# LiMeng95/MultiPoseNet.pytorch

Hardware: AMD Instinct MI355X
Metric: images/sec (train fwd+bwd) ResNet101 480x480 bs=32/GPU (higher is better)
Workload: dtype bf16; 1 GPU; R101 full posenet (keypoint+detection) train step: fwd + MSE/focal losses + bwd + Adam, 480x480, 32 images/GPU, bf16 MFMA / fp32 accumulate / fp32 master weights; global_batch=32, parallelism=dp1, loss_log=asynchronous (set_lazy_log), launch=recorded launch list re-issued per step (replay.py), 88 replays, optimizer_update=Adam in one launch after backward

## Files before the change

include/mpn.h:

```cpp
#ifndef MPN_H_
#define MPN_H_
#include <stdint.h>

#ifdef __cplusplus
extern "C" {
#endif

#define MPN_F32 0
#define MPN_BF16 1
#define MPN_F16 2

#define MPN_E_BADARG (-2)
#define MPN_E_UNSUPPORTED (-3)

typedef struct MpnConvParams {
    const void* x;
    const void* w;
    void* y;
    const float* bias;
    const float* scale;
    const void* res;
    const uint8_t* res_mask;
    float* stats;
    int64_t x_sB, x_sH, x_sW;
// ... 73 lines not shown
} MpnWgradParams;
int mpn_debug_wgrad_prof(void* buf);
int mpn_debug_igemm_prof(void* buf);

int mpn_conv_wgrad_chunks(const MpnWgradParams* p);
int mpn_conv_wgrad_seg_plan(MpnWgradParams* p);
int mpn_conv_wgrad(const MpnWgradParams* p, void* stream);
int mpn_conv_wgrad_partials(const MpnWgradParams* p, void* stream);
int mpn_conv_wgrad_reduce(const MpnWgradParams* p, void* stream);
int mpn_conv_wgrad_kernel_id(const MpnWgradParams* p);

int mpn_reduce_partials(const float* ws, int chunks, int64_t n, float* dst, int accumulate, void* stream);

int mpn_cast_f32_to_bf16(const float* src, void* dst, int64_t n, void* stream);
int mpn_cast_f32(const float* src, void* dst, int64_t n, int dtype, void* stream);
int mpn_weight_transpose(const float* w, void* wt, int Cout, int RS, int Cin, int Cout_pad,
                         int dtype, void* stream);
int mpn_weight_transpose_batched(const float* arena, void* dst, const int64_t* table, int nlayers, int64_t nblocks,
                                 int dtype, void* stream);
int mpn_weight_pad_k(const float* w, void* dst, int Cout, int K, int Kpad, int dtype, void* stream);
int mpn_stem_pack_weight(const float* w, void* packed, int Cout, int dtype, void* stream);
int mpn_stem_unpack_wgrad(const float* dpacked, float* dw, int Cout, void* stream);
int mpn_stem_pack_image(const float* img, int64_t sB, int64_t sC, int64_t sH, int64_t sW, void* dst,
                        int B, int H, int W, int dtype, void* stream);

int mpn_bn_finalize_train(const float* stats, int tiles, int C, int64_t count, const float* gamma,
                          const float* beta, float* running_mean, float* running_var, float momentum,
                          float eps, float* mean, float* invstd, float* scale, float* shift, void* stream);
int mpn_bn_finalize_eval(int C, const float* gamma, const float* beta, const float* running_mean,
                         const float* running_var, float eps, float* mean, float* invstd,
                         float* scale, float* shift, void* stream);
int mpn_bn_act_forward(const void* y, const void* res, void* z, const float* scale, const float* shift,
                       int64_t P, int C, int Cs, int relu, int dtype, uint8_t* mask, void* stream);
int mpn_bn_bwd_reduce(const void* dz, const void* z, const void* y, const float* mean, const float* invstd,
                      const float* mask_scale, const float* mask_shift, float* partial, int chunks, int64_t P, int C, int Cs, int relu, int dtype, void* stream);
int mpn_bn_bwd_finalize(const float* partial, int chunks, int C, int64_t count, const float* gamma, const float* mean,
                        const float* invstd, int train, float* dgamma, float* dbeta, float* coef, void* stream);
int mpn_bn_bwd_apply(const void* dz, const void* z, const void* y, const float* k1, const float* k2, const float* k3,
                     const float* mask_scale, const float* mask_shift, void* dy, void* dres, int dres_accumulate, int64_t P, int C, int Cs, int relu, int dtype,
                     const uint8_t* mask, void* stream);
int mpn_bn_bwd_chunks(int64_t P, int Cs, int dtype);

int mpn_maxpool3x3s2_forward(const void* x, void* y, uint8_t* idx, int B, int H, int W, int Cs,
                             int Ho, int Wo, int dtype, void* stream);
int mpn_maxpool3x3s2_backward(const void* dy, const uint8_t* idx, void* dx, int B, int H, int W, int Cs,
                              int Ho, int Wo, int dtype, void* stream);
int mpn_upsample_nearest_backward(const void* dfine, void* dcoarse, int B, int Hf, int Wf, int Hc, int Wc,
                                  int Cs, int accumulate, int dtype, void* stream);
int mpn_upsample_nearest_slice(const void* src, void* dst, int B, int Hs, int Ws, int Cs_src,
                               int Ho, int Wo, int Cs_dst, int c_off, int dtype, void* stream);
int mpn_upsample_nearest_slice_backward(const void* ddst, void* dsrc, int B, int Hs, int Ws, int Cs_src,
                                        int Ho, int Wo, int Cs_dst, int c_off, int dtype, void* stream);
int mpn_export_f32(const void* src, int src_dtype, float* dst, int B, int Hs, int Ws, int Cs, int C,
                   int Ho, int Wo, int64_t dst_sB, int64_t dst_sP, void* stream);
int mpn_import_grad(const float* ddst, int64_t ddst_sB, int64_t ddst_sP, void* dsrc, int dst_dtype,
                    int B, int Hs, int Ws, int Cs, int C, int Ho, int Wo, void* stream);
int mpn_nchw_to_nhwc_f32(const float* src, int64_t sB, int64_t sC, int64_t sH, int64_t sW, float* dst,
                         int B, int C, int H, int W, void* stream);
int mpn_det_pack(const void* src, int src_dtype, float* dst, int B, int64_t HW, int Cs, int C, int64_t dst_sB, void* stream);
int mpn_det_unpack(const float* ddst, void* dsrc, int dst_dtype, int B, int64_t HW, int Cs, int C, int64_t dst_sB, void* stream);
int mpn_relu_forward(const void* x, void* y, int64_t n, int dtype, void* stream);
int mpn_relu_backward(const void* dz, const void* z, void* dx, int64_t n, int accumulate, int dtype, void* stream);
int mpn_add_inplace(void* dst, const void* src, int64_t n, int dtype, void* stream);
int mpn_channel_sum(const void* dy, int dy_dtype, int64_t P, int C, int Cs, float* partial, int chunks, void* stream);
int mpn_channel_sum_chunks(int64_t P, int Cs, int dtype);
int mpn_colsum_rows(const void* dy, int dy_dtype, int64_t P, int C, int Cs, float* db, void* stream);
// ... 112 lines not shown
```

multiposenet/pytorch_amd/_lib.py:

```python
import ctypes
import os
import subprocess

import torch

_HERE = os.path.dirname(os.path.abspath(__file__))
LIB_PATH = os.path.join(_HERE, "libmpn_hip.so")
CSRC = os.path.join(_HERE, "csrc")

F32, BF16, F16 = 0, 1, 2


class MpnError(RuntimeError):
    pass


class ConvParams(ctypes.Structure):
    _fields_ = [
        ("x", ctypes.c_void_p), ("w", ctypes.c_void_p), ("y", ctypes.c_void_p),
        ("bias", ctypes.c_void_p), ("scale", ctypes.c_void_p), ("res", ctypes.c_void_p), ("res_mask", ctypes.c_void_p),
        ("stats", ctypes.c_void_p),
        ("x_sB", ctypes.c_int64), ("x_sH", ctypes.c_int64), ("x_sW", ctypes.c_int64),
        ("y_sB", ctypes.c_int64), ("y_sP", ctypes.c_int64),
        ("res_sB", ctypes.c_int64), ("res_sP", ctypes.c_int64),
# ... 38 lines not shown
SIGNATURES = {
    "mpn_gt_heatmaps": (_i, [_vp, _vp, _i, _i, _vp, _i, _i, ctypes.c_double, ctypes.c_double, _vp]),
    "mpn_heatmap_peaks_workspace_bytes": (_i64, [_i, _i, _i, _i, _i]),
    "mpn_heatmap_peaks": (_i, [_vp, _i64, _i64, _i64, _i64, _i, _i, _i, _i, _f, ctypes.c_double, _i, _vp, _vp, _i, _vp, _vp]),
    "mpn_resize": (_i, [_vp, _i64, _i64, _i64, _i, _i, _i, _vp, _i, _i, _i, ctypes.c_double, ctypes.c_double, _vp]),
    "mpn_prn_build_maps": (_i, [_vp, _vp, _vp, _vp, _i, _i, _i, ctypes.c_double, _vp, _vp, _vp, _vp, _vp]),
    "mpn_prn_scores": (_i, [_vp, _vp, _i, _i, _i, _i, _vp, _vp, _vp]),
    "mpn_prn_scores_compact": (_i, [_vp, _vp, _i, _i, _i, _i, _i, _vp, _vp, _vp, _vp, _vp, _vp]),
    "mpn_prn_match_host": (_i, [_i, _vp, _vp, _vp, _vp, _vp, _vp, _vp, _i, _vp, _i, _i, _vp, _vp]),
    "mpn_conv_stats_tiles": (_i, [_PC]),
    "mpn_conv_tile_rows": (_i, [_PC]),
    "mpn_conv_shared_tile": (_i, [_PC]),
    "mpn_conv_forward": (_i, [_PC, _vp]),
    "mpn_debug_wgrad_prof": (_i, [_vp]),
    "mpn_debug_igemm_prof": (_i, [_vp]),
    "mpn_conv_wgrad_chunks": (_i, [_PW]),
    "mpn_conv_wgrad_seg_plan": (_i, [_PW]),
    "mpn_conv_wgrad": (_i, [_PW, _vp]),
    "mpn_conv_wgrad_partials": (_i, [_PW, _vp]),
    "mpn_conv_wgrad_reduce": (_i, [_PW, _vp]),
    "mpn_conv_wgrad_kernel_id": (_i, [_PW]),
    "mpn_reduce_partials": (_i, [_vp, _i, _i64, _vp, _i, _vp]),
    "mpn_cast_f32_to_bf16": (_i, [_vp, _vp, _i64, _vp]),
    "mpn_cast_f32": (_i, [_vp, _vp, _i64, _i, _vp]),
    "mpn_weight_transpose": (_i, [_vp, _vp, _i, _i, _i, _i, _i, _vp]),
    "mpn_weight_transpose_batched": (_i, [_vp, _vp, _vp, _i, _i64, _i, _vp]),
    "mpn_weight_pad_k": (_i, [_vp, _vp, _i, _i, _i, _i, _vp]),
    "mpn_stem_pack_weight": (_i, [_vp, _vp, _i, _i, _vp]),
    "mpn_stem_unpack_wgrad": (_i, [_vp, _vp, _i, _vp]),
    "mpn_stem_pack_image": (_i, [_vp, _i64, _i64, _i64, _i64, _vp, _i, _i, _i, _i, _vp]),
    "mpn_bn_finalize_train": (_i, [_vp, _i, _i, _i64, _vp, _vp, _vp, _vp, _f, _f, _vp, _vp, _vp, _vp, _vp]),
    "mpn_bn_finalize_eval": (_i, [_i, _vp, _vp, _vp, _vp, _f, _vp, _vp, _vp, _vp, _vp]),
    "mpn_bn_act_forward": (_i, [_vp, _vp, _vp, _vp, _vp, _i64, _i, _i, _i, _i, _vp, _vp]),
    "mpn_bn_bwd_reduce": (_i, [_vp, _vp, _vp, _vp, _vp, _vp, _vp, _vp, _i, _i64, _i, _i, _i, _i, _vp]),
    "mpn_bn_bwd_finalize": (_i, [_vp, _i, _i, _i64, _vp, _vp, _vp, _i, _vp, _vp, _vp, _vp]),
    "mpn_bn_bwd_apply": (_i, [_vp, _vp, _vp, _vp, _vp, _vp, _vp, _vp, _vp, _vp, _i, _i64, _i, _i, _i, _i, _vp, _vp]),
    "mpn_bn_bwd_chunks": (_i, [_i64, _i, _i]),
    "mpn_maxpool3x3s2_forward": (_i, [_vp, _vp, _vp, _i, _i, _i, _i, _i, _i, _i, _vp]),
    "mpn_maxpool3x3s2_backward": (_i, [_vp, _vp, _vp, _i, _i, _i, _i, _i, _i, _i, _vp]),
    "mpn_upsample_nearest_backward": (_i, [_vp, _vp, _i, _i, _i, _i, _i, _i, _i, _i, _vp]),
    "mpn_upsample_nearest_slice": (_i, [_vp, _vp, _i, _i, _i, _i, _i, _i, _i, _i, _i, _vp]),
    "mpn_upsample_nearest_slice_backward": (_i, [_vp, _vp, _i, _i, _i, _i, _i, _i, _i, _i, _i, _vp]),
    "mpn_export_f32": (_i, [_vp, _i, _vp, _i, _i, _i, _i, _i, _i, _i, _i64, _i64, _vp]),
    "mpn_import_grad": (_i, [_vp, _i64, _i64, _vp, _i, _i, _i, _i, _i, _i, _i, _i, _vp]),
    "mpn_nchw_to_nhwc_f32": (_i, [_vp, _i64, _i64, _i64, _i64, _vp, _i, _i, _i, _i, _vp]),
    "mpn_det_pack": (_i, [_vp, _i, _vp, _i, _i64, _i, _i, _i64, _vp]),
    "mpn_det_unpack": (_i, [_vp, _vp, _i, _i, _i64, _i, _i, _i64, _vp]),
    "mpn_relu_forward": (_i, [_vp, _vp, _i64, _i, _vp]),
    "mpn_relu_backward": (_i, [_vp, _vp, _vp, _i64, _i, _i, _vp]),
    "mpn_add_inplace": (_i, [_vp, _vp, _i64, _i, _vp]),
    "mpn_channel_sum": (_i, [_vp, _i, _i64, _i, _i, _vp, _i, _vp]),
    "mpn_colsum_rows": (_i, [_vp, _i, _i64, _i, _i, _vp, _vp]),
    "mpn_channel_sum_chunks": (_i, [_i64, _i, _i]),
    "mpn_mse_chunks": (_i, [_i64]),
    "mpn_mse_heatmap_forward": (_i, [_vp, _vp, _vp, _vp, _i64, _vp, _i, _vp, _vp]),
    "mpn_mse_heatmap_backward": (_i, [_vp, _vp, _vp, _vp, _vp, _vp, _vp, _i64, _vp, _vp]),
    "mpn_mse_train_blocks": (_i, [_i, _i, _i]),
    "mpn_mse_heatmap_train": (_i, [_vp, _vp, _vp, _i, _vp, _vp, _i64, _i64, _i64, _i, _i, _i, _vp, _vp, _i, _vp, _vp]),
    "mpn_focal_blocks": (_i, [_i]),
    "mpn_focal_forward": (_i, [_vp, _vp, _vp, _vp, _i, _i, _i, _vp, _vp, _vp, _vp]),
    "mpn_focal_backward": (_i, [_vp, _vp, _vp, _vp, _i, _i, _i, _vp, _vp, _vp, _vp, _vp]),
    "mpn_focal_mc_blocks": (_i, [_i]),
    "mpn_focal_forward_mc": (_i, [_vp, _vp, _vp, _vp, _i, _i, _i, _i, _vp, _vp, _vp, _vp, _vp]),
    "mpn_focal_backward_mc": (_i, [_vp, _vp, _vp, _vp, _i, _i, _i, _i, _vp, _vp, _vp, _vp, _vp]),
    "mpn_class_max": (_i, [_vp, _i, _i, _i, _vp, _vp, _vp]),
    "mpn_sigmoid_forward": (_i, [_vp, _vp, _i64, _vp]),
# ... 117 lines not shown
```

multiposenet/pytorch_amd/csrc/bn.hip:

```cpp
#include "common.h"
#include <stdlib.h>

namespace {

template <typename T> struct Geo {
    static constexpr int V = Vec16<T>::N;
    int G, GB, lanes, g, pl, c0;
    __device__ __forceinline__ Geo(int Cs) {
        G = Cs / V;
        GB = G < 256 ? G : 256;
        lanes = 256 / GB;
        g = blockIdx.y * GB + (threadIdx.x % GB);
        pl = threadIdx.x / GB;
        c0 = g * V;
    }
};

template <int V>
__device__ __forceinline__ void load_coef(const float* __restrict__ p, int c0, int C, float (&out)[V], float fill) {
#pragma unroll
    for (int k = 0; k < V; k += 4) {
        if (p != nullptr && c0 + k + 3 < C) {
            const float4 t = *reinterpret_cast<const float4*>(p + c0 + k);
            out[k] = t.x; out[k + 1] = t.y; out[k + 2] = t.z; out[k + 3] = t.w;
        } else {
#pragma unroll
            for (int j = 0; j < 4; ++j) out[k + j] = (p != nullptr && c0 + k + j < C) ? p[c0 + k + j] : fill;
        }
    }
}

__device__ __forceinline__ void reduce_slices(const float* __restrict__ part, int n, int C, int c, int sl, double& s1, double& s2) {
    const float* col = part + (long)c * 2;
    const long stride = (long)C * 2;
    int t = sl;
    for (; t + 7 * 64 < n; t += 8 * 64) {
        float2 v[8];
#pragma unroll
        for (int u = 0; u < 8; ++u) v[u] = *reinterpret_cast<const float2*>(col + (long)(t + u * 64) * stride);
#pragma unroll
        for (int u = 0; u < 8; ++u) { s1 += (double)v[u].x; s2 += (double)v[u].y; }
    }
    float2 w[8];
    int m = 0;
#pragma unroll
    for (int u = 0; u < 8; ++u) {
        const int tt = t + u * 64;
        w[u] = tt < n ? *reinterpret_cast<const float2*>(col + (long)tt * stride) : make_float2(0.f, 0.f);
        m += tt < n ? 1 : 0;
    }
#pragma unroll
    for (int u = 0; u < 8; ++u) if (u < m) { s1 += (double)w[u].x; s2 += (double)w[u].y; }
}

__device__ __forceinline__ void finalize_train_block(int blk, const float* __restrict__ stats, int tiles, int C, double count,
                                                     const float* __restrict__ gamma, const float* __restrict__ beta,
                                                     float* __restrict__ rm, float* __restrict__ rv, float momentum, float eps,
                                                     float* __restrict__ mean, float* __restrict__ invstd,
                                                     float* __restrict__ scale, float* __restrict__ shift, double (*sh)[4][4]) {
    const int cl = threadIdx.x & 3, sl = threadIdx.x >> 2;
    const int c = blk * 4 + cl;
    double s1 = 0.0, s2 = 0.0;
    const bool fin = sl == 0 && c < C;
    const float g = (fin && gamma) ? gamma[c] : 1.f, b = (fin && beta) ? beta[c] : 0.f;
    const float rm0 = (fin && rm) ? rm[c] : 0.f, rv0 = (fin && rv) ? rv[c] : 0.f;
    if (c < C) reduce_slices(stats, tiles, C, c, sl, s1, s2);
#pragma unroll
    for (int m = 4; m < 64; m <<= 1) { s1 += __shfl_xor(s1, m); s2 += __shfl_xor(s2, m); }
    const int lane = threadIdx.x & 63, wave = threadIdx.x >> 6;
    if (lane < 4) { sh[0][wave][cl] = s1; sh[1][wave][cl] = s2; }
    __syncthreads();
    if (sl == 0 && c < C) {
        s1 = (sh[0][0][cl] + sh[0][1][cl]) + (sh[0][2][cl] + sh[0][3][cl]);
        s2 = (sh[1][0][cl] + sh[1][1][cl]) + (sh[1][2][cl] + sh[1][3][cl]);
        const double mu = s1 / count;
        double var = s2 / count - mu * mu;
        if (var < 0.0) var = 0.0;
        const float is = (float)(1.0 / sqrt(var + (double)eps));
        const float sc = g * is;
        mean[c] = (float)mu; invstd[c] = is;
        scale[c] = sc; shift[c] = b - (float)mu * sc;
        if (rm) rm[c] = (1.f - momentum) * rm0 + momentum * (float)mu;
        if (rv) {
            const double unb = count > 1.0 ? var * count / (count - 1.0) : var;
            rv[c] = (1.f - momentum) * rv0 + momentum * (float)unb;
        }
    }
}

__global__ void bn_finalize_train_kernel(const float* __restrict__ stats, int tiles, int C, double count,
                                         const float* __restrict__ gamma, const float* __restrict__ beta,
                                         float* __restrict__ rm, float* __restrict__ rv, float momentum, float eps,
                                         float* __restrict__ mean, float* __restrict__ invstd,
                                         float* __restrict__ scale, float* __restrict__ shift) {
    __shared__ double sh[2][4][4];
    finalize_train_block(blockIdx.x, stats, tiles, C, count, gamma, beta, rm, rv, momentum, eps, mean, invstd, scale, shift, sh);
}

__global__ void bn_finalize_eval_kernel(int C, const float* __restrict__ gamma, const float* __restrict__ beta,
                                        const float* __restrict__ rm, const float* __restrict__ rv, float eps,
                                        float* __restrict__ mean, float* __restrict__ invstd,
                                        float* __restrict__ scale, float* __restrict__ shift) {
    const int c = blockIdx.x * blockDim.x + threadIdx.x;
    if (c >= C) return;
    const float is = 1.0f / sqrtf(rv[c] + eps);
    const float sc = gamma[c] * is;
    mean[c] = rm[c]; invstd[c] = is; scale[c] = sc; shift[c] = beta[c] - rm[c] * sc;
}

template <typename T>
__global__ void __launch_bounds__(256) bn_act_kernel(const T* __restrict__ y, const T* __restrict__ res, T* __restrict__ z,
                                                     const float* __restrict__ scale, const float* __restrict__ shift,
                                                     long P, int C, int Cs, int relu, int iters, unsigned char* __restrict__ mask) {
    constexpr int V = Vec16<T>::N;
    const Geo<T> q(Cs);
    float sc[V], sf[V];
    load_coef<V>(scale, q.c0, C, sc, 0.f);
    load_coef<V>(shift, q.c0, C, sf, 0.f);
    const long p0 = (long)blockIdx.x * q.lanes * iters + q.pl;
    for (int it = 0; it < iters; ++it) {
        const long p = p0 + (long)it * q.lanes;
        if (p >= P) break;
        const long off = p * Cs + q.c0;
        Vec16<T> a; a.load(y + off);
        Vec16<T> r;
        if (res) r.load(res + off);
#pragma unroll
        for (int k = 0; k < V; ++k) {
            float x = a.v[k] * sc[k] + sf[k];
            if (res) x += r.v[k];
            if (relu) x = fmaxf(x, 0.f);
            a.v[k] = (q.c0 + k < C) ? x : 0.f;
        }
        a.store(z + off);
        if (mask) {
            unsigned bits = 0;
#pragma unroll
            for (int k = 0; k < V; ++k) bits |= (Elem<T>::round(a.v[k]) > 0.f ? 1u : 0u) << k;
            mask[p * q.G + q.g] = (unsigned char)bits;
        }
    }
}

template <typename T>
__global__ void __launch_bounds__(256) bn_bwd_reduce_kernel(const T* __restrict__ dz, const T* __restrict__ z, const T* __restrict__ y,
                                                            const float* __restrict__ mean, const float* __restrict__ invstd,
                                                            const float* __restrict__ mscale, const float* __restrict__ mshift,
                                                            float* __restrict__ partial, long P, int C, int Cs, int relu, int chunk_pix) {
    constexpr int V = Vec16<T>::N;
    __shared__ float sh[256][2 * V + 1];
    const Geo<T> q(Cs);
    const long p_begin = (long)blockIdx.x * chunk_pix;
    long p_end = p_begin + chunk_pix; if (p_end > P) p_end = P;
    float s1[V], s2[V], mu[V], is[V], sc[V], sf[V];
    load_coef<V>(mean, q.c0, C, mu, 0.f);
    load_coef<V>(invstd, q.c0, C, is, 0.f);
    const bool remask = relu && z == nullptr;
    if (remask) { load_coef<V>(mscale, q.c0, C, sc, 0.f); load_coef<V>(mshift, q.c0, C, sf, 0.f); }
#pragma unroll
    for (int k = 0; k < V; ++k) { s1[k] = 0.f; s2[k] = 0.f; }
    for (long p = p_begin + q.pl; p < p_end; p += q.lanes) {
        const long off = p * Cs + q.c0;
        Vec16<T> d, o, x;
        d.load(dz + off); x.load(y + off);
        if (relu && !remask) o.load(z + off);
#pragma unroll
        for (int k = 0; k < V; ++k) {
            float gk = d.v[k];
            if (remask) o.v[k] = x.v[k] * sc[k] + sf[k];
            if (relu && !(o.v[k] > 0.f)) gk = 0.f;
            s1[k] += gk;
            s2[k] += gk * ((x.v[k] - mu[k]) * is[k]);
        }
// ... 113 lines not shown

}

extern "C" int mpn_bn_finalize_train(const float* stats, int tiles, int C, int64_t count, const float* gamma,
                                     const float* beta, float* running_mean, float* running_var, float momentum,
                                     float eps, float* mean, float* invstd, float* scale, float* shift, void* stream) {
    MPN_CHECK_ARG(stats && tiles > 0 && C > 0 && count > 0 && mean && invstd && scale && shift);
    hipLaunchKernelGGL(bn_finalize_train_kernel, dim3((C + 3) / 4), dim3(256), 0, (hipStream_t)stream, stats, tiles, C,
                       (double)count, gamma, beta, running_mean, running_var, momentum, eps, mean, invstd, scale, shift);
    return mpn_launch_status();
}

extern "C" int mpn_bn_finalize_eval(int C, const float* gamma, const float* beta, const float* running_mean,
                                    const float* running_var, float eps, float* mean, float* invstd,
                                    float* scale, float* shift, void* stream) {
    MPN_CHECK_ARG(C > 0 && gamma && beta && running_mean && running_var && mean && invstd && scale && shift);
    hipLaunchKernelGGL(bn_finalize_eval_kernel, dim3((C + 255) / 256), dim3(256), 0, (hipStream_t)stream, C, gamma, beta,
                       running_mean, running_var, eps, mean, invstd, scale, shift);
    return mpn_launch_status();
}

extern "C" int mpn_bn_act_forward(const void* y, const void* res, void* z, const float* scale, const float* shift,
                                  int64_t P, int C, int Cs, int relu, int dtype, uint8_t* mask, void* stream) {
    MPN_CHECK_ARG(y && z && scale && shift && P > 0 && C > 0 && Cs >= C && (!mask || relu));
    const int V = dtype == MPN_F32 ? 4 : 8;
    MPN_CHECK_ARG(geo_ok(Cs, V) && C % 4 == 0);
    const int lanes = geo_lanes(Cs, V), iters = pick_iters(P, lanes);
    dim3 grid((unsigned)((P + (long)lanes * iters - 1) / ((long)lanes * iters)), (unsigned)geo_yblocks(Cs, V));
    MPN_DISPATCH_T(dtype, hipLaunchKernelGGL((bn_act_kernel<T>), grid, dim3(256), 0, (hipStream_t)stream, (const T*)y, (const T*)res,
                           (T*)z, scale, shift, (long)P, C, Cs, relu, iters, (unsigned char*)mask));
    return mpn_launch_status();
}

extern "C" int mpn_bn_bwd_chunks(int64_t P, int Cs, int dtype) {
    const int V = dtype == MPN_F32 ? 4 : 8;
    if (!geo_ok(Cs, V) || P <= 0) return MPN_E_BADARG;
    const int chunk = reduce_chunk(P, geo_lanes(Cs, V));
    return (int)((P + chunk - 1) / chunk);
}

extern "C" int mpn_bn_bwd_reduce(const void* dz, const void* z, const void* y, const float* mean, const float* invstd,
                                 const float* mask_scale, const float* mask_shift, float* partial, int chunks, int64_t P, int C, int Cs, int relu, int dtype, void* stream) {
    MPN_CHECK_ARG(dz && y && mean && invstd && partial && P > 0 && C > 0 && Cs >= C);
    MPN_CHECK_ARG(!relu || z || (mask_scale && mask_shift && y));
    const int V = dtype == MPN_F32 ? 4 : 8;
    MPN_CHECK_ARG(geo_ok(Cs, V) && C % 4 == 0);
    const int chunk = reduce_chunk(P, geo_lanes(Cs, V));
    MPN_CHECK_ARG(chunks == (int)((P + chunk - 1) / chunk));
    dim3 grid((unsigned)chunks, (unsigned)geo_yblocks(Cs, V));
    MPN_DISPATCH_T(dtype, hipLaunchKernelGGL((bn_bwd_reduce_kernel<T>), grid, dim3(256), 0, (hipStream_t)stream, (const T*)dz, (const T*)z,
                           (const T*)y, mean, invstd, mask_scale, mask_shift, partial, (long)P, C, Cs, relu, chunk));
    return mpn_launch_status();
}

extern "C" int mpn_bn_bwd_finalize(const float* partial, int chunks, int C, int64_t count, const float* gamma, const float* mean,
                                   const float* invstd, int train, float* dgamma, float* dbeta, float* coef, void* stream) {
    MPN_CHECK_ARG(partial && chunks > 0 && C > 0 && count > 0);
    MPN_CHECK_ARG(!coef || (mean && invstd));
    hipLaunchKernelGGL(bn_bwd_finalize_kernel, dim3((C + 3) / 4), dim3(256), 0, (hipStream_t)stream, partial, chunks, C,
                       (double)count, gamma, mean, invstd, train, dgamma, dbeta, coef);
    return mpn_launch_status();
}

extern "C" int mpn_bn_bwd_apply(const void* dz, const void* z, const void* y, const float* k1, const float* k2, const float* k3,
                                const float* mask_scale, const float* mask_shift, void* dy, void* dres, int dres_accumulate, int64_t P, int C, int Cs, int relu, int dtype,
                                const uint8_t* mask, void* stream) {
// ... 14 lines not shown
```

multiposenet/pytorch_amd/engine.py:

```python
import ctypes
import os

import torch

from . import ops
from ._lib import MpnError, call, gpu_op
from .ops import Act, round_up


class Ctx(object):

    def __init__(self, train):
        self.train = train
        self.tape = []
        self.grads = {}
        self.keep = []
        self.out_grads = {}
        self.wt = {}
        self.wt_buf = None
        self.uses = {}
        self.bn_train_ran = False
        self.side_keep = []
        self.side_pending = []
        self.wt_ready = None
# ... 19 lines not shown
        self.grads[id(act)] = g
        self.keep.append(act)

    def pop_grad(self, act):
        return self.grads.pop(id(act), None)


def num_classes(cm):
    cout = cm.output.weight.shape[0]
    if cout % 9 != 0 or cout == 0 or getattr(cm, "num_anchors", 9) != 9:
        raise MpnError("classificationModel: the output convolution has %d channels; the detector needs 9 anchors x K classes" % cout)
    return cout // 9


def _geom(layer):
    w = layer.weight
    if w.dim() == 2:
        return w.shape[0], w.shape[1], 1, 1, 1, 0
    return w.shape[0], w.shape[1], w.shape[2], w.shape[3], layer.stride[0], layer.padding[0]


class Engine(object):
    def __init__(self, model):
        self.m = model
        self._drop_calls = 0
        self._side = None
        self._wt_plan_cache = None
        self.overlap_wgrad = os.environ.get("MPN_SIDE_STREAM", "1") != "0"
        self.fork_every = max(1, int(os.environ.get("MPN_SIDE_FORK_EVERY", "1")))
        self.pyramid_towers = os.environ.get("MPN_PYRAMID_TOWERS", "1") != "0"
        self.fuse_bn_stats = os.environ.get("MPN_BN_FUSED_STATS", "1") != "0"
        self.fold_bn = os.environ.get("MPN_FOLD_BN", "1") != "0"
        self.fuse_bn_finalize = os.environ.get("MPN_BN_FUSED_FINALIZE", "1") != "0"
        self.det_pyramid_side = int(os.environ.get("MPN_DET_PYRAMID_SIDE", "2"))
        self.bn_mask_bits = os.environ.get("MPN_BN_MASK_BITS", "1") != "0"
        self.defer_shortcut_grad = os.environ.get("MPN_DEFER_SHORTCUT_GRAD", "1") != "0"
        self.virtual_concat = os.environ.get("MPN_VIRTUAL_CONCAT", "1") != "0"
        self.conv2_classes = os.environ.get("MPN_CONV2_CLASSES", "1") != "0"

    def side_stream(self, device):
        if not self.overlap_wgrad or device.type != "cuda":
            return None
        if self._side is None:
            self._side = torch.cuda.Stream(device=device)
        return self._side

    def _on_side(self, ctx, device, keep, fn, torch_ops=False):
        side = self.side_stream(device)
        if side is None:
            fn()
            return
        ctx.side_keep.append(keep)
        ctx.side_pending.append((fn, torch_ops))
        if len(ctx.side_pending) >= self.fork_every:
            self.flush_side(ctx, device)

    def flush_side(self, ctx, device):
        if not ctx.side_pending:
            return
        side = self.side_stream(device)
        pending, ctx.side_pending = ctx.side_pending, []
        ev = torch.cuda.Event()
        gpu_op(ev.record, torch.cuda.current_stream(device))
        gpu_op(side.wait_event, ev)
        for fn, torch_ops in pending:
            if torch_ops:
# ... 256 lines not shown
                if wg:
                    handled, fused = ops.conv_wgrad_seg(xs, dys, ar.grad_seg(layer.weight), O, R, S, pad, db=ar.grad_seg(bias) if bg else None)
                for x, d in zip(xs, dys):
                    done = fused
                    if wg and not handled:
                        done = ops.conv_wgrad(x, d, ar.grad_seg(layer.weight), O, R, S, 1, pad, db=ar.grad_seg(bias) if bg else None)
                    if bg and not done:
                        ops.bias_grad(d, ar.grad_seg(bias), O)
            self._on_side(ctx, dys[0].t.device, (xs, dys), param_grads)
            if wg:
                self._grad_done(ctx, layer.weight)
            if bg:
                self._grad_done(ctx, bias)
        if any(x.needs_grad for x in xs):
            wt = self.w_t(ctx, layer)
            grouped = ops.seg_flat(xs) is not None
            if grouped and ctx.grad_of(xs[0]) is None:
                gs = ops.alloc_seg(xs, xs[0].C, xs[0].t.dtype)
                for x, g in zip(xs, gs):
                    ctx.set_grad(x, g)
                existed = [False] * len(xs)
            else:
                pairs = [ctx.gbuf(x) for x in xs]
                gs, existed = [g for g, _ in pairs], [e for _, e in pairs]
            if all(existed) or not any(existed):
                ops.conv_forward_seg(dys, wt, I, R, S, pad, mode=1, cin=wt.shape[3], outs=gs, accumulate=existed[0])
            else:
                for d, x, g, e in zip(dys, xs, gs, existed):
                    ops.conv_forward(d, wt, I, R, S, 1, pad, mode=1, out_hw=(x.H, x.W), cin=wt.shape[3], out=g, accumulate=e)

    def bn(self, ctx, y, stats, layer, relu, res=None, tag=""):
        train_stats = layer.training
        want_mask = bool(self.bn_mask_bits and ctx.train and relu and res is not None)
        if train_stats:
            momentum = layer.momentum if layer.momentum is not None else 0.1
            if isinstance(stats, ops.BNState):
                st = stats
            else:
                st = ops.bn_finalize_train(stats, y.P, layer.weight.data, layer.bias.data, layer.running_mean, layer.running_var,
                                           momentum, layer.eps)
            ctx.bn_train_ran = True
        else:
            st = ops.bn_finalize_eval(layer.weight.data, layer.bias.data, layer.running_mean, layer.running_var, layer.eps)
        z = ops.bn_act(y, st, relu, res=res, tag=tag, want_mask=want_mask)
        if ctx.train:
            z.needs_grad = bool(y.needs_grad or layer.weight.requires_grad or layer.bias.requires_grad
                                or (res is not None and res.needs_grad))
            if z.needs_grad:
                self._note_use(ctx, layer.weight)
                self._note_use(ctx, layer.bias)
                if res is not None and res.needs_grad:
                    res.cons += 1
                    res.other_cons += 1
                wants_stats = bool(train_stats or layer.weight.requires_grad or layer.bias.requires_grad)
                z.bn_src = (y, st, relu, res is not None, wants_stats, layer, train_stats)
                ctx.tape.append(lambda: self._bn_bwd(ctx, y, z, st, layer, relu, res, train_stats))
        return z

    @staticmethod
    def _bnb_args(fused):
        if fused is None:
            return {}
        if isinstance(fused, str) or (fused.dim() == 2 and fused.shape[0] == 3):
            return {"coef": fused}
        return {"partial": fused}

    def _bn_bwd(self, ctx, y, z, st, layer, relu, res, train_stats):
        dz = ctx.pop_grad(z)
        wg, bg = layer.weight.requires_grad, layer.bias.requires_grad
        if dz is None:
            if wg:
                self._grad_done(ctx, layer.weight)
            if bg:
                self._grad_done(ctx, layer.bias)
            if res is not None and res.needs_grad:
                res.cons -= 1
            return
# ... 552 lines not shown
```

multiposenet/pytorch_amd/ops.py:

```python
import ctypes
import os

import torch

from . import _lib
from ._lib import BF16, F16, F32, ConvParams, WgradParams, call


def round_up(v, m):
    return (v + m - 1) // m * m


def dtype_code(dt):
    if dt == torch.float32:
        return F32
    if dt == torch.bfloat16:
        return BF16
    if dt == torch.float16:
        return F16
    raise _lib.MpnError("unsupported dtype %s" % dt)


_STREAM_OVERRIDE = []

# ... 661 lines not shown
class BNState(object):
    __slots__ = ("mean", "invstd", "scale", "shift")

    def __init__(self, C, device):
        buf = torch.empty((4, C), dtype=torch.float32, device=device)
        self.mean, self.invstd, self.scale, self.shift = buf[0], buf[1], buf[2], buf[3]


def bn_finalize_train(stats, count, gamma, beta, rm, rv, momentum=0.1, eps=1e-5):
    C = stats.shape[1]
    st = BNState(C, stats.device)
    call("mpn_bn_finalize_train", ptr(stats), stats.shape[0], C, count, ptr(gamma), ptr(beta), ptr(rm), ptr(rv),
         momentum, eps, ptr(st.mean), ptr(st.invstd), ptr(st.scale), ptr(st.shift), stream_ptr())
    return st


def bn_finalize_eval(gamma, beta, rm, rv, eps=1e-5):
    C = gamma.numel()
    st = BNState(C, gamma.device)
    call("mpn_bn_finalize_eval", C, ptr(gamma), ptr(beta), ptr(rm), ptr(rv), eps, ptr(st.mean), ptr(st.invstd),
         ptr(st.scale), ptr(st.shift), stream_ptr())
    return st


def bn_act(y, st, relu, res=None, needs_grad=False, tag="", want_mask=False):
    z = Act(torch.empty_like(y.t), y.C, needs_grad, tag)
    if want_mask and relu:
        z.mask = torch.empty((y.P, y.Cs // (4 if y.t.dtype == torch.float32 else 8)), dtype=torch.uint8, device=y.t.device)
    call("mpn_bn_act_forward", ptr(y.t), ptr(res.t) if res is not None else None, ptr(z.t), ptr(st.scale), ptr(st.shift),
         y.P, y.C, y.Cs, 1 if relu else 0, dtype_code(y.t.dtype), ptr(z.mask), stream_ptr())
    return z


def masked_copy(dz, mask_bits, out):
    call("mpn_bn_bwd_apply", ptr(dz.t), None, None, None, None, None, None, None, None, ptr(out.t), 0, dz.P, dz.C, dz.Cs, 1,
         dtype_code(dz.t.dtype), ptr(mask_bits), stream_ptr())
    return out


def bn_backward(dz, z, y, st, gamma, relu, train, dgamma=None, dbeta=None, want_dy=True, dres=None, dres_acc=False, remask=False,
                partial=None, coef=None):
    dev = y.t.device
    P, C, Cs = y.P, y.C, y.Cs
    dc = dtype_code(y.t.dtype)
    k1, k2, k3 = st.scale, None, None
    if coef is not None:
        if not isinstance(coef, str):
            k1, k2, k3 = coef[0], coef[1], coef[2]
    elif train or dgamma is not None or dbeta is not None:
        if partial is not None:
            part, chunks = partial, partial.shape[0]
        else:
            chunks = call("mpn_bn_bwd_chunks", P, Cs, dc)
            part = workspace(chunks * C * 2 * 4, dev, slot=3)
            call("mpn_bn_bwd_reduce", ptr(dz.t), ptr(z.t) if (relu and not remask) else None, ptr(y.t), ptr(st.mean), ptr(st.invstd),
                 ptr(st.scale) if remask else None, ptr(st.shift) if remask else None, ptr(part),
                 chunks, P, C, Cs, 1 if relu else 0, dc, stream_ptr())
        coef = torch.empty((3, C), dtype=torch.float32, device=dev) if train else None
        call("mpn_bn_bwd_finalize", ptr(part), chunks, C, P, ptr(gamma), ptr(st.mean), ptr(st.invstd), 1 if train else 0,
             ptr(dgamma), ptr(dbeta), ptr(coef), stream_ptr())
        if train:
            k1, k2, k3 = coef[0], coef[1], coef[2]
    dy = None
    if want_dy or dres is not None:
        if want_dy:
            dy = Act(torch.empty_like(y.t), C)
# ... 219 lines not shown
```

Before: 892.9 images/sec.

## Fuse BN train finalize into BN activation kernel for mid-size tile counts

Result: no change. 894.1 images/sec (median of 6 runs) (+0.1%).

```diff
diff --git a/include/mpn.h b/include/mpn.h
--- a/include/mpn.h
+++ b/include/mpn.h
@@ -129,6 +129,10 @@
                          float* scale, float* shift, void* stream);
 int mpn_bn_act_forward(const void* y, const void* res, void* z, const float* scale, const float* shift,
                        int64_t P, int C, int Cs, int relu, int dtype, uint8_t* mask, void* stream);
+int mpn_bn_act_train(const float* stats, int tiles, int C, int64_t count, const float* gamma, const float* beta,
+                     float* running_mean, float* running_var, float momentum, float eps, float* mean, float* invstd,
+                     float* scale, float* shift, const void* y, const void* res, void* z, int relu, uint8_t* mask,
+                     int64_t P, int Cs, int dtype, void* stream);
 int mpn_bn_bwd_reduce(const void* dz, const void* z, const void* y, const float* mean, const float* invstd,
                       const float* mask_scale, const float* mask_shift, float* partial, int chunks, int64_t P, int C, int Cs, int relu, int dtype, void* stream);
 int mpn_bn_bwd_finalize(const float* partial, int chunks, int C, int64_t count, const float* gamma, const float* mean,
diff --git a/multiposenet/pytorch_amd/_lib.py b/multiposenet/pytorch_amd/_lib.py
--- a/multiposenet/pytorch_amd/_lib.py
+++ b/multiposenet/pytorch_amd/_lib.py
@@ -94,6 +94,8 @@
     "mpn_bn_finalize_train": (_i, [_vp, _i, _i, _i64, _vp, _vp, _vp, _vp, _f, _f, _vp, _vp, _vp, _vp, _vp]),
     "mpn_bn_finalize_eval": (_i, [_i, _vp, _vp, _vp, _vp, _f, _vp, _vp, _vp, _vp, _vp]),
     "mpn_bn_act_forward": (_i, [_vp, _vp, _vp, _vp, _vp, _i64, _i, _i, _i, _i, _vp, _vp]),
+    "mpn_bn_act_train": (_i, [_vp, _i, _i, _i64, _vp, _vp, _vp, _vp, _f, _f, _vp, _vp, _vp, _vp, _vp, _vp, _vp, _i, _vp, _i64, _i, _i,
+                              _vp]),
     "mpn_bn_bwd_reduce": (_i, [_vp, _vp, _vp, _vp, _vp, _vp, _vp, _vp, _i, _i64, _i, _i, _i, _i, _vp]),
     "mpn_bn_bwd_finalize": (_i, [_vp, _i, _i, _i64, _vp, _vp, _vp, _i, _vp, _vp, _vp, _vp]),
     "mpn_bn_bwd_apply": (_i, [_vp, _vp, _vp, _vp, _vp, _vp, _vp, _vp, _vp, _vp, _i, _i64, _i, _i, _i, _i, _vp, _vp]),
diff --git a/multiposenet/pytorch_amd/csrc/bn.hip b/multiposenet/pytorch_amd/csrc/bn.hip
--- a/multiposenet/pytorch_amd/csrc/bn.hip
+++ b/multiposenet/pytorch_amd/csrc/bn.hip
@@ -30,27 +30,62 @@
     }
 }
 
-__device__ __forceinline__ void reduce_slices(const float* __restrict__ part, int n, int C, int c, int sl, double& s1, double& s2) {
+template <int NC, int ROWS>
+__device__ __forceinline__ void reduce_slices(const float* __restrict__ part, int n, int C, int c, int sl, double (&s1)[NC],
+                                              double (&s2)[NC]) {
     const float* col = part + (long)c * 2;
     const long stride = (long)C * 2;
     int t = sl;
-    for (; t + 7 * 64 < n; t += 8 * 64) {
-        float2 v[8];
-#pragma unroll
-        for (int u = 0; u < 8; ++u) v[u] = *reinterpret_cast<const float2*>(col + (long)(t + u * 64) * stride);
-#pragma unroll
-        for (int u = 0; u < 8; ++u) { s1 += (double)v[u].x; s2 += (double)v[u].y; }
-    }
-    float2 w[8];
+    for (; t + (ROWS - 1) * 64 < n; t += ROWS * 64) {
+        float2 v[ROWS][NC];
+#pragma unroll
+        for (int u = 0; u < ROWS; ++u)
+#pragma unroll
+            for (int i = 0; i < NC; ++i) v[u][i] = *reinterpret_cast<const float2*>(col + (long)(t + u * 64) * stride + 2 * i);
+#pragma unroll
+        for (int u = 0; u < ROWS; ++u)
+#pragma unroll
+            for (int i = 0; i < NC; ++i) { s1[i] += (double)v[u][i].x; s2[i] += (double)v[u][i].y; }
+    }
+    float2 w[ROWS][NC];
     int m = 0;
 #pragma unroll
-    for (int u = 0; u < 8; ++u) {
+    for (int u = 0; u < ROWS; ++u) {
         const int tt = t + u * 64;
-        w[u] = tt < n ? *reinterpret_cast<const float2*>(col + (long)tt * stride) : make_float2(0.f, 0.f);
+#pragma unroll
+        for (int i = 0; i < NC; ++i) w[u][i] = tt < n ? *reinterpret_cast<const float2*>(col + (long)tt * stride + 2 * i) : make_float2(0.f, 0.f);
         m += tt < n ? 1 : 0;
     }
 #pragma unroll
-    for (int u = 0; u < 8; ++u) if (u < m) { s1 += (double)w[u].x; s2 += (double)w[u].y; }
+    for (int u = 0; u < ROWS; ++u)
+        if (u < m) {
+#pragma unroll
+            for (int i = 0; i < NC; ++i) { s1[i] += (double)w[u][i].x; s2[i] += (double)w[u][i].y; }
+        }
+}
+
+__device__ __forceinline__ void reduce_slices(const float* __restrict__ part, int n, int C, int c, int sl, double& s1, double& s2) {
+    double a[1] = {s1}, b[1] = {s2};
+    reduce_slices<1, 8>(part, n, C, c, sl, a, b);
+    s1 = a[0]; s2 = b[0];
+}
+
+struct BnTrainCoef { float mean, invstd, scale, shift, rm, rv; };
+__device__ __forceinline__ BnTrainCoef bn_train_coef(double s1, double s2, double count, float g, float b, float rm0, float rv0,
+                                                     float momentum, float eps) {
+#pragma clang fp contract(off)
+    BnTrainCoef r;
+    const double mu = s1 / count;
+    double var = fma(-mu, mu, s2 / count);
+    if (var < 0.0) var = 0.0;
+    const float is = (float)(1.0 / sqrt(var + (double)eps));
+    const float sc = g * is;
+    r.mean = (float)mu; r.invstd = is;
+    r.scale = sc; r.shift = fmaf(-(float)mu, sc, b);
+    r.rm = (1.f - momentum) * rm0 + momentum * (float)mu;
+    const double unb = count > 1.0 ? var * count / (count - 1.0) : var;
+    r.rv = (1.f - momentum) * rv0 + momentum * (float)unb;
+    return r;
 }
 
 __device__ __forceinline__ void finalize_train_block(int blk, const float* __restrict__ stats, int tiles, int C, double count,
@@ -73,18 +108,11 @@
     if (sl == 0 && c < C) {
         s1 = (sh[0][0][cl] + sh[0][1][cl]) + (sh[0][2][cl] + sh[0][3][cl]);
         s2 = (sh[1][0][cl] + sh[1][1][cl]) + (sh[1][2][cl] + sh[1][3][cl]);
-        const double mu = s1 / count;
-        double var = s2 / count - mu * mu;
-        if (var < 0.0) var = 0.0;
-        const float is = (float)(1.0 / sqrt(var + (double)eps));
-        const float sc = g * is;
-        mean[c] = (float)mu; invstd[c] = is;
-        scale[c] = sc; shift[c] = b - (float)mu * sc;
-        if (rm) rm[c] = (1.f - momentum) * rm0 + momentum * (float)mu;
-        if (rv) {
-            const double unb = count > 1.0 ? var * count / (count - 1.0) : var;
-            rv[c] = (1.f - momentum) * rv0 + momentum * (float)unb;
-        }
+        const BnTrainCoef k = bn_train_coef(s1, s2, count, g, b, rm0, rv0, momentum, eps);
+        mean[c] = k.mean; invstd[c] = k.invstd;
+        scale[c] = k.scale; shift[c] = k.shift;
+        if (rm) rm[c] = k.rm;
+        if (rv) rv[c] = k.rv;
     }
 }
 
@@ -106,6 +134,26 @@
     const float is = 1.0f / sqrtf(rv[c] + eps);
     const float sc = gamma[c] * is;
     mean[c] = rm[c]; invstd[c] = is; scale[c] = sc; shift[c] = beta[c] - rm[c] * sc;
+}
+
+template <typename T, int V>
+__device__ __forceinline__ void bn_act_chunk(Vec16<T>& a, const Vec16<T>& r, bool has_res, int relu, const float (&sc)[V],
+                                             const float (&sf)[V], int c0, int C) {
+#pragma unroll
+    for (int k = 0; k < V; ++k) {
+        float x = a.v[k] * sc[k] + sf[k];
+        if (has_res) x += r.v[k];
+        if (relu) x = fmaxf(x, 0.f);
+        a.v[k] = (c0 + k < C) ? x : 0.f;
+    }
+}
+
+template <typename T, int V>
+__device__ __forceinline__ unsigned char chunk_sign_bits(const Vec16<T>& a) {
+    unsigned bits = 0;
+#pragma unroll
+    for (int k = 0; k < V; ++k) bits |= (Elem<T>::round(a.v[k]) > 0.f ? 1u : 0u) << k;
+    return (unsigned char)bits;
 }
 
 template <typename T>
@@ -125,20 +173,109 @@
         Vec16<T> a; a.load(y + off);
         Vec16<T> r;
         if (res) r.load(res + off);
-#pragma unroll
-        for (int k = 0; k < V; ++k) {
-            float x = a.v[k] * sc[k] + sf[k];
-            if (res) x += r.v[k];
-            if (relu) x = fmaxf(x, 0.f);
-            a.v[k] = (q.c0 + k < C) ? x : 0.f;
-        }
+        bn_act_chunk<T, V>(a, r, res != nullptr, relu, sc, sf, q.c0, C);
         a.store(z + off);
-        if (mask) {
-            unsigned bits = 0;
-#pragma unroll
-            for (int k = 0; k < V; ++k) bits |= (Elem<T>::round(a.v[k]) > 0.f ? 1u : 0u) << k;
-            mask[p * q.G + q.g] = (unsigned char)bits;
-        }
+        if (mask) mask[p * q.G + q.g] = chunk_sign_bits<T, V>(a);
+    }
+}
+
+constexpr int kTrainSlice = 64;
+constexpr int kTrainThreads = 1024;
+constexpr int kTrainUnroll = 2;
+
+template <typename T>
+__global__ void __launch_bounds__(kTrainThreads) bn_act_train_kernel(
+        const float* __restrict__ stats, int tiles, int C, double count, const float* __restrict__ gamma,
+        const float* __restrict__ beta, float* __restrict__ rm, float* __restrict__ rv, float momentum, float eps,
+        float* __restrict__ mean, float* __restrict__ invstd, float* __restrict__ scale, float* __restrict__ shift,
+        const T* __restrict__ y, const T* __restrict__ res, T* __restrict__ z, long P, int Cs, int relu, long ppb,
+        unsigned char* __restrict__ mask) {
+    constexpr int V = Vec16<T>::N;
+    constexpr int NC = kTrainSlice / 16;
+    __shared__ double sh[2][4][kTrainSlice];
+    __shared__ float coef[2][kTrainSlice];
+    const int tid = threadIdx.x;
+    const int cbase = blockIdx.y * kTrainSlice;
+    const bool owner = blockIdx.x == 0;
+    constexpr int GB = kTrainSlice / V, LANES = kTrainThreads / GB;
+    constexpr long STEP = (long)LANES * kTrainUnroll;
+    const int gl = tid % GB, pl = tid / GB;
+    const int c0 = cbase + gl * V;
+    const long pbeg = (long)blockIdx.x * ppb;
+    const long pend = pbeg + ppb < P ? pbeg + ppb : P;
+    Vec16<T> a[kTrainUnroll], r[kTrainUnroll];
+    long p = pbeg + pl;
+#pragma unroll
+    for (int u = 0; u < kTrainUnroll; ++u) {
+        const long pu = p + (long)u * LANES;
+        if (pu < pend) a[u].load(y + pu * Cs + c0);
+    }
+    const int cf = cbase + tid;
+    const bool fin = tid < kTrainSlice && cf < C;
+    const float g = (fin && gamma) ? gamma[cf] : 1.f, b = (fin && beta) ? beta[cf] : 0.f;
+    const float rm0 = (fin && owner && rm) ? rm[cf] : 0.f, rv0 = (fin && owner && rv) ? rv[cf] : 0.f;
+    {
+        const int cl = tid & 3, sl = (tid >> 2) & 63, j = tid >> 8;
+        const int lc = j * 16 + cl * NC;
+        double s1[NC], s2[NC];
+#pragma unroll
+        for (int i = 0; i < NC; ++i) { s1[i] = 0.0; s2[i] = 0.0; }
+        if (cbase + lc < C) reduce_slices<NC, 4>(stats, tiles, C, cbase + lc, sl, s1, s2);
+#pragma unroll
+        for (int i = 0; i < NC; ++i) {
+#pragma unroll
+            for (int m = 4; m < 64; m <<= 1) { s1[i] += __shfl_xor(s1[i], m); s2[i] += __shfl_xor(s2[i], m); }
+        }
+        if ((tid & 63) < 4) {
+#pragma unroll
+            for (int i = 0; i < NC; ++i) { sh[0][sl >> 4][lc + i] = s1[i]; sh[1][sl >> 4][lc + i] = s2[i]; }
+        }
+    }
+    __syncthreads();
+    if (tid < kTrainSlice) {
+        float sc = 0.f, sf = 0.f;
+        if (cf < C) {
+            const double s1 = (sh[0][0][tid] + sh[0][1][tid]) + (sh[0][2][tid] + sh[0][3][tid]);
+            const double s2 = (sh[1][0][tid] + sh[1][1][tid]) + (sh[1][2][tid] + sh[1][3][tid]);
+            const BnTrainCoef k = bn_train_coef(s1, s2, count, g, b, rm0, rv0, momentum, eps);
+            sc = k.scale; sf = k.shift;
+            if (owner) {
+                mean[cf] = k.mean; invstd[cf] = k.invstd;
+                scale[cf] = k.scale; shift[cf] = k.shift;
+                if (rm) rm[cf] = k.rm;
+                if (rv) rv[cf] = k.rv;
+            }
+        }
+        coef[0][tid] = sc; coef[1][tid] = sf;
+    }
+    __syncthreads();
+    float sc[V], sf[V];
+#pragma unroll
+    for (int k = 0; k < V; ++k) { sc[k] = coef[0][gl * V + k]; sf[k] = coef[1][gl * V + k]; }
+    const long G = Cs / V, gidx = c0 / V;
+    for (; p < pend; p += STEP) {
+        Vec16<T> an[kTrainUnroll];
+#pragma unroll
+        for (int u = 0; u < kTrainUnroll; ++u) {
+            const long pu = p + STEP + (long)u * LANES;
+            if (pu < pend) an[u].load(y + pu * Cs + c0);
+        }
+        if (res) {
+#pragma unroll
+            for (int u = 0; u < kTrainUnroll; ++u)
+                if (p + (long)u * LANES < pend) r[u].load(res + (p + (long)u * LANES) * Cs + c0);
+        }
+#pragma unroll
+        for (int u = 0; u < kTrainUnroll; ++u) {
+            const long pu = p + (long)u * LANES;
+            if (pu < pend) {
+                bn_act_chunk<T, V>(a[u], r[u], res != nullptr, relu, sc, sf, c0, C);
+                a[u].store(z + pu * Cs + c0);
+                if (mask) mask[pu * G + gidx] = chunk_sign_bits<T, V>(a[u]);
+            }
+        }
+#pragma unroll
+        for (int u = 0; u < kTrainUnroll; ++u) a[u] = an[u];
     }
 }
 
@@ -318,6 +455,24 @@
     return mpn_launch_status();
 }
 
+extern "C" int mpn_bn_act_train(const float* stats, int tiles, int C, int64_t count, const float* gamma, const float* beta,
+                                float* running_mean, float* running_var, float momentum, float eps, float* mean, float* invstd,
+                                float* scale, float* shift, const void* y, const void* res, void* z, int relu, uint8_t* mask,
+                                int64_t P, int Cs, int dtype, void* stream) {
+    MPN_CHECK_ARG(stats && tiles > 0 && C > 0 && count > 0 && mean && invstd && scale && shift);
+    MPN_CHECK_ARG(y && z && P > 0 && Cs >= C && C % 4 == 0 && Cs % kTrainSlice == 0 && (!mask || relu) && mpn_dtype_ok(dtype));
+    static const long blocks = mpn_tune("MPN_BN_TRAIN_BLOCKS", 256);
+    const long ny = Cs / kTrainSlice;
+    long ranges = (blocks + ny - 1) / ny;
+    if (ranges < 1) ranges = 1;
+    const long ppb = (P + ranges - 1) / ranges;
+    dim3 grid((unsigned)((P + ppb - 1) / ppb), (unsigned)ny);
+    MPN_DISPATCH_T(dtype, hipLaunchKernelGGL((bn_act_train_kernel<T>), grid, dim3(kTrainThreads), 0, (hipStream_t)stream, stats, tiles, C,
+                           (double)count, gamma, beta, running_mean, running_var, momentum, eps, mean, invstd, scale, shift,
+                           (const T*)y, (const T*)res, (T*)z, (long)P, Cs, relu, ppb, (unsigned char*)mask));
+    return mpn_launch_status();
+}
+
 extern "C" int mpn_bn_bwd_chunks(int64_t P, int Cs, int dtype) {
     const int V = dtype == MPN_F32 ? 4 : 8;
     if (!geo_ok(Cs, V) || P <= 0) return MPN_E_BADARG;
diff --git a/multiposenet/pytorch_amd/engine.py b/multiposenet/pytorch_amd/engine.py
--- a/multiposenet/pytorch_amd/engine.py
+++ b/multiposenet/pytorch_amd/engine.py
@@ -75,6 +75,7 @@
         self.fuse_bn_stats = os.environ.get("MPN_BN_FUSED_STATS", "1") != "0"
         self.fold_bn = os.environ.get("MPN_FOLD_BN", "1") != "0"
         self.fuse_bn_finalize = os.environ.get("MPN_BN_FUSED_FINALIZE", "1") != "0"
+        self.bn_act_train = os.environ.get("MPN_BN_ACT_TRAIN", "1") != "0"
         self.det_pyramid_side = int(os.environ.get("MPN_DET_PYRAMID_SIDE", "2"))
         self.bn_mask_bits = os.environ.get("MPN_BN_MASK_BITS", "1") != "0"
         self.defer_shortcut_grad = os.environ.get("MPN_DEFER_SHORTCUT_GRAD", "1") != "0"
@@ -397,17 +398,22 @@
     def bn(self, ctx, y, stats, layer, relu, res=None, tag=""):
         train_stats = layer.training
         want_mask = bool(self.bn_mask_bits and ctx.train and relu and res is not None)
+        z = None
         if train_stats:
             momentum = layer.momentum if layer.momentum is not None else 0.1
             if isinstance(stats, ops.BNState):
                 st = stats
+            elif self.bn_act_train and ops.bn_act_train_ok(y, stats):
+                z, st = ops.bn_act_train(y, stats, layer.weight.data, layer.bias.data, layer.running_mean, layer.running_var, momentum,
+                                         layer.eps, relu, res=res, tag=tag, want_mask=want_mask)
             else:
                 st = ops.bn_finalize_train(stats, y.P, layer.weight.data, layer.bias.data, layer.running_mean, layer.running_var,
                                            momentum, layer.eps)
             ctx.bn_train_ran = True
         else:
             st = ops.bn_finalize_eval(layer.weight.data, layer.bias.data, layer.running_mean, layer.running_var, layer.eps)
-        z = ops.bn_act(y, st, relu, res=res, tag=tag, want_mask=want_mask)
+        if z is None:
+            z = ops.bn_act(y, st, relu, res=res, tag=tag, want_mask=want_mask)
         if ctx.train:
             z.needs_grad = bool(y.needs_grad or layer.weight.requires_grad or layer.bias.requires_grad
                                 or (res is not None and res.needs_grad))
diff --git a/multiposenet/pytorch_amd/ops.py b/multiposenet/pytorch_amd/ops.py
--- a/multiposenet/pytorch_amd/ops.py
+++ b/multiposenet/pytorch_amd/ops.py
@@ -717,6 +717,27 @@
     return z
 
 
+BN_ACT_TRAIN_MAX_TILES = 256
+BN_ACT_TRAIN_MAX_C = 512
+
+
+def bn_act_train_ok(y, stats):
+    return (FIN_MAX_TILES < stats.shape[0] <= BN_ACT_TRAIN_MAX_TILES and stats.shape[1] == y.C <= BN_ACT_TRAIN_MAX_C
+            and y.Cs % 64 == 0 and y.C % 4 == 0)
+
+
+def bn_act_train(y, stats, gamma, beta, rm, rv, momentum, eps, relu, res=None, needs_grad=False, tag="", want_mask=False):
+    C = stats.shape[1]
+    st = BNState(C, stats.device)
+    z = Act(torch.empty_like(y.t), y.C, needs_grad, tag)
+    if want_mask and relu:
+        z.mask = torch.empty((y.P, y.Cs // (4 if y.t.dtype == torch.float32 else 8)), dtype=torch.uint8, device=y.t.device)
+    call("mpn_bn_act_train", ptr(stats), stats.shape[0], C, y.P, ptr(gamma), ptr(beta), ptr(rm), ptr(rv), momentum, eps,
+         ptr(st.mean), ptr(st.invstd), ptr(st.scale), ptr(st.shift), ptr(y.t), ptr(res.t) if res is not None else None, ptr(z.t),
+         1 if relu else 0, ptr(z.mask), y.P, y.Cs, dtype_code(y.t.dtype), stream_ptr())
+    return z, st
+
+
 def masked_copy(dz, mask_bits, out):
     call("mpn_bn_bwd_apply", ptr(dz.t), None, None, None, None, None, None, None, None, ptr(out.t), 0, dz.P, dz.C, dz.Cs, 1,
          dtype_code(dz.t.dtype), ptr(mask_bits), stream_ptr())
```
